# sandyresearch/chipmunk

Measured on AMD Instinct MI355X. Metric: DiT denoise steps/sec at fixed sparsity, higher is better.
Workload: dtype bf16

## Files before the change

### chipmunk_amd/csrc/attn64.hip

```cpp
#include "common.h"
#include "attn64_regs.h"
#include "attn_params.h"
#include "attn64_util.h"
#include <type_traits>

namespace {

constexpr int HD = 128;
constexpr int KT = 64;
constexpr int WROWS = 64, WGROWS = 256;
constexpr int TB = KT * HD * 2;
constexpr int NSL = 4;
constexpr int VRING = NSL * TB;
constexpr int LDS_BYTES = 2 * NSL * TB;
constexpr int PSTAGE = 64 * 128;
constexpr int LDS_BYTES_CSUM = LDS_BYTES + 4 * PSTAGE;
constexpr int CS_EXCH_BYTES = 2 * 4 * 64 * 4;
constexpr float SCALE_LOG2E = 0.08838834764f * 1.44269504089f;
constexpr float MAX_LAG = 4.0f;
#ifndef A64_ABL
#define A64_ABL 0
#endif
#ifndef A64_EB
#define A64_EB 20
#endif
#ifndef A64_EA
#define A64_EA 35
#endif
#ifndef A64_CSUM_VALU
#define A64_CSUM_VALU 1
#endif
#ifndef A64_VSPREAD
#define A64_VSPREAD 0
#endif
#ifndef A64_DMA_POS
#define A64_DMA_POS 2
#endif

constexpr int a64_ecum(int k) {
    return k <= 0 ? 0 : k <= 20 ? (k * A64_EB) / 20 : k <= 52 ? A64_EB + ((k - 20) * A64_EA) / 32
                                                              : (A64_EB + A64_EA + (k - 52) < 64 ? A64_EB + A64_EA + (k - 52) : 64);
}
constexpr int a64_cstep(int j) {
    int k = 0;
    while (a64_ecum(k) < 2 * j + 2) ++k;
    return k;
}
constexpr int a64_rk(int u) { return u == 0 ? 36 : u == 1 ? 38 : u == 2 ? 68 : 70; }
constexpr int a64_mk(int u) { return u == 0 ? 46 : u == 1 ? 48 : u == 2 ? 78 : 80; }

#ifdef ATTN64_PROF
__device__ unsigned long long g_a64_prof[4 * 8];
#define P64_DECL unsigned long long pt_ = 0, pacc_[7] = {0, 0, 0, 0, 0, 0, 0}; const bool prof_on_ = blockIdx.x == (gridDim.x / 2)
#define P64_START() do { if (prof_on_) pt_ = __builtin_amdgcn_s_memtime(); } while (0)
#define P64_MARK(i) do { if (prof_on_) { const unsigned long long n_ = __builtin_amdgcn_s_memtime(); pacc_[i] += n_ - pt_; pt_ = n_; } } while (0)
#define P64_END(w, n) do { if (prof_on_ && lane == 0) { for (int i_ = 0; i_ < 7; ++i_) g_a64_prof[(w) * 8 + i_] = pacc_[i_]; g_a64_prof[(w) * 8 + 7] = (n); } } while (0)
#else
#define P64_DECL
#define P64_START()
#define P64_MARK(i)
#define P64_END(w, n)
#endif

template <int KB, int QB, int KS>
__device__ __forceinline__ void mfma_qk(f32x16 &s) {
    constexpr int ka = 192 + (KB * 8 + KS) * 4, qa = 128 + (QB * 8 + KS) * 4;
    if constexpr (A64_ABL & 64) {
        constexpr int oa = (KB * 2 + QB) * 16;
        asm volatile("v_mfma_f32_32x32x16_bf16 a[%c0:%c1], a[%c2:%c3], a[%c4:%c5], a[%c0:%c1]" ::"i"(oa), "i"(oa + 15), "i"(ka), "i"(ka + 3), "i"(qa), "i"(qa + 3));
        return;
    }
    if constexpr (KS == 0)
        asm volatile("v_mfma_f32_32x32x16_bf16 %0, a[%c1:%c2], a[%c3:%c4], 0" : "=v"(s) : "i"(ka), "i"(ka + 3), "i"(qa), "i"(qa + 3));
    else
        asm volatile("v_mfma_f32_32x32x16_bf16 %0, a[%c1:%c2], a[%c3:%c4], %0" : "+v"(s) : "i"(ka), "i"(ka + 3), "i"(qa), "i"(qa + 3));
}
template <int QB, int DB>
__device__ __forceinline__ void mfma_pv(const u32x4 &vf, const u32x4 &pf) {
    constexpr int oa = (QB * 4 + DB) * 16;
    asm volatile("v_mfma_f32_32x32x16_bf16 a[%c2:%c3], %0, %1, a[%c2:%c3]" ::"v"(vf), "v"(pf), "i"(oa), "i"(oa + 15));
}
template <int KB, int KS, int SLOT>
__device__ __forceinline__ void lds_k(uint32_t addr) {
    constexpr int ka = 192 + (KB * 8 + KS) * 4;
    asm volatile("ds_read_b128 a[%c1:%c2], %0 offset:%c3" ::"v"(addr), "i"(ka), "i"(ka + 3), "i"(SLOT * TB + KB * 8192) : "memory");
}
__device__ __forceinline__ void cs_pair16x2(float &a, float &b, float &c, float &d) {
    asm volatile("v_permlane16_swap_b32 %0, %1\n\tv_permlane16_swap_b32 %2, %3\n\tv_add_f32 %0, %0, %1\n\tv_add_f32 %2, %2, %3"
                 : "+v"(a), "+v"(b), "+v"(c), "+v"(d));
}
__device__ __forceinline__ void cs_pair8(float &a, const float &b) {
    asm volatile("v_add_f32_dpp %0, %0, %0 row_mirror row_mask:0xf bank_mask:0x3\n\t"
                 "v_add_f32_dpp %0, %1, %1 row_mirror row_mask:0xf bank_mask:0xc" : "+v"(a) : "v"(b));
}
__device__ __forceinline__ void cs_pair4(float &a, const float &b) {
    asm volatile("v_add_f32_dpp %0, %0, %0 row_half_mirror row_mask:0xf bank_mask:0x5\n\t"
                 "v_add_f32_dpp %0, %1, %1 row_half_mirror row_mask:0xf bank_mask:0xa" : "+v"(a) : "v"(b));
}
template <int CTRL>
__device__ __forceinline__ float cs_pair_quad(float a, float b, bool hi) {
    const float keep = hi ? b : a, give = hi ? a : b;
    return keep + __uint_as_float((uint32_t)__builtin_amdgcn_update_dpp(0, (int)__float_as_uint(give), CTRL, 0xf, 0xf, true));
}
__global__ __launch_bounds__(256) void knorm_max_kernel(const uint16_t *k, const int64_t ks0, const int64_t ks1, const int64_t ks2, int H, int Nk,
                                                        float *out) {
    const int bh = blockIdx.y, b = bh / H, h = bh - b * H;
    const uint16_t *kb = k + b * ks0 + h * ks1;
    const int grp = threadIdx.x >> 4, li = threadIdx.x & 15;
    float best = 0.f;
#pragma unroll 4
    for (int row = blockIdx.x * 16 + grp; row < Nk; row += gridDim.x * 16) {
        const u32x4 v = *(const u32x4 *)(kb + (int64_t)row * ks2 + li * 8);
        float ss = 0.f;
#pragma unroll
        for (int e = 0; e < 4; ++e) {
            const float lo = __uint_as_float(v[e] << 16), hi = __uint_as_float(v[e] & 0xffff0000u);
            ss = __builtin_fmaf(lo, lo, ss);
            ss = __builtin_fmaf(hi, hi, ss);
        }
        best = fmaxf(best, row16_sum(ss));
    }
    __shared__ float red[256];
    red[threadIdx.x] = best;
    __syncthreads();
    for (int st = 128; st > 0; st >>= 1) {
        if ((int)threadIdx.x < st) red[threadIdx.x] = fmaxf(red[threadIdx.x], red[threadIdx.x + st]);
        __syncthreads();
    }
    if (threadIdx.x == 0) atomicMax((unsigned int *)(out + bh), __float_as_uint(__builtin_sqrtf(red[0])));
}

template <int MODE>
// ... 96 lines not shown
            __syncthreads();
        }
        return;
    }

    asm volatile(A64_ZERO_O ::: A64_CLOBBER_ALL);
    float qss[2] = {0.f, 0.f};
    {
        const uint16_t *qp = p.q + b * p.qs[0] + h * p.qs[1];
        static_for<0, 16>([&](auto f) {
            constexpr int F = decltype(f)::value, qb = F >> 3, ks = F & 7;
            const int qrow = row0 + qb * 32 + l31;
            u32x4 val = {0u, 0u, 0u, 0u};
            if (qrow < p.Nq) val = *(const u32x4 *)(qp + (int64_t)qrow * p.qs[2] + ks * 16 + hf * 8);
            acc_write4<128 + F * 4>(val);
#pragma unroll
            for (int e = 0; e < 4; ++e) {
                const float lo = __uint_as_float(val[e] << 16), hi = __uint_as_float(val[e] & 0xffff0000u);
                qss[qb] = __builtin_fmaf(lo, lo, qss[qb]);
                qss[qb] = __builtin_fmaf(hi, hi, qss[qb]);
            }
        });
    }

    const uint32_t lds0 = (uint32_t)(uintptr_t)(__attribute__((address_space(3))) unsigned char *)smem;
    uint32_t kad[8];
#pragma unroll
    for (int ks = 0; ks < 8; ++ks) kad[ks] = lds0 + l31 * 256 + (((2 * ks + hf) ^ l15) << 4);
    uint32_t vad[4];
#pragma unroll
    for (int db = 0; db < 4; ++db)
        vad[db] = lds0 + VRING + (4 * hf + (l15 >> 2)) * 256 + (((db * 4 + 2 * (lg & 1) + ((l15 & 3) >> 1)) ^ ((l15 >> 2) << 2)) << 4) +
                  (l15 & 1) * 8;
    uint32_t kofs[4];
#pragma unroll
    for (int i = 0; i < 4; ++i) kofs[i] = (uint32_t)(w * 16 + 4 * i + lg) * kstride_b + ((uint32_t)(l15 ^ (4 * i + lg)) << 4);
    const uint32_t vofs = (uint32_t)(w * 16 + lg) * vstride_b + ((uint32_t)(l15 ^ (lg << 2)) << 4);

    const int last_base = p.Nk - KT;
    auto tile_base = [&](int T) { return T * KT < last_base ? T * KT : last_base; };
    auto issue_k1 = [&](uint32_t soff, uint32_t ldsw, int slot, int i) {
        blds16(krsrc, kofs[i], soff, smem + ldsw + slot * TB + i * 1024);
    };
    auto issue_v1 = [&](uint32_t soff, uint32_t ldsw, int slot, int i) {
        blds16(vrsrc, vofs, soff + (uint32_t)(4 * i) * vstride_b, smem + ldsw + VRING + slot * TB + i * 1024);
    };
    auto issue_k = [&](int T, int slot) {
        const uint32_t soff = (uint32_t)tile_base(T) * kstride_b;
#pragma unroll
        for (int i = 0; i < 4; ++i) issue_k1(soff, w * 4096, slot, i);
    };
    auto issue_v = [&](int T, int slot) {
        const uint32_t soff = (uint32_t)tile_base(T) * vstride_b;
#pragma unroll
        for (int i = 0; i < 4; ++i) issue_v1(soff, w * 4096, slot, i);
    };

    if constexpr (!GATHER) {
        issue_k(0, 0);
        issue_k(1, 1), issue_v(0, 3);
        issue_k(2, 2), issue_v(0, 0);
        issue_k(3, 3), issue_v(1, 1);
        asm volatile("s_waitcnt vmcnt(24)" ::: "memory");
    }
    __syncthreads();
    static_for<0, 16>([&](auto i) {
        constexpr int I = decltype(i)::value;
        lds_k<(I >> 3), (I & 7), 0>(kad[I & 7]);
    });
    asm volatile("s_waitcnt lgkmcnt(0)" ::: "memory");

    f32x16 s[4];
    float px[64];
    uint32_t pw[2][4][4] = {};
    float m[2] = {-INFINITY, -INFINITY}, nmsc[2] = {0.f, 0.f};
    float mlag[2] = {-INFINITY, -INFINITY};
    float lacc[2][2] = {{0.f, 0.f}, {0.f, 0.f}};
    float alpha[2] = {1.f, 1.f};
    float wq[2] = {0.f, 0.f}, lpq[2] = {-1.0e30f, -1.0e30f}, c4[2] = {0.f, 0.f}, c5 = 0.f;
    uint32_t csoff = 0, ex_w = 0, ex_r = 0;
    int cs_extra = 0;
    float cs_own = 0.f;
    __amdgpu_buffer_rsrc_t prsrc = krsrc;
    uint32_t pst_w = 0, pst_r = 0, csoff_mx = 0;
    u32x2 csf[8] = {};
    f32x4 csacc[2] = {{0.f, 0.f, 0.f, 0.f}, {0.f, 0.f, 0.f, 0.f}};
    float csout = 0.f;
    u32x4 cs_ones = {0x3f803f80u, 0x3f803f80u, 0x3f803f80u, 0x3f803f80u};
    if constexpr (CSUM) {
        static_assert(A64_CSUM_VALU, "the matrix-pipe column-sum probe (A64_CSUM_VALU=0) fills all 160 KiB of LDS with its P stage: no room for the exchange area of the in-workgroup combine; build round 5's tree for it");
        pin(cs_ones);
        const uint32_t pst = lds0 + LDS_BYTES + (uint32_t)w * PSTAGE;
        pst_w = pst + l31 * 128 + ((uint32_t)(hf ^ (l31 & 7)) << 4);
        const int prow = lg * 4 + (l15 >> 2);
        pst_r = pst + prow * 128 + ((uint32_t)(((l15 & 3) >> 1) ^ (prow & 7)) << 4) + (l15 & 1) * 8;
        csoff_mx = 2u * (uint32_t)(16 * lg + 8 * ((l15 >> 2) & 1) + 4 * (l15 >> 3) + (l15 & 3));
#pragma unroll
        for (int qb = 0; qb < 2; ++qb) {
            const int qrow = row0 + qb * 32 + l31;
            const float pl = qrow < p.Nq ? p.p_in[(int64_t)bh * p.Nq + qrow] : 0.f;
            lpq[qb] = pl > 0.f ? __builtin_amdgcn_logf(pl) : -1.0e30f;
        }
        const int rr = ((lane >> 4) & 1) | (((lane >> 3) & 1) << 1) | (((lane >> 2) & 1) << 2);
        csoff = 2u * (uint32_t)(32 * (lane & 1) + (rr & 3) + 8 * (2 * ((lane >> 1) & 1) + (rr >> 2)) + 4 * hf);
        const int nA = 3 - (4 * g) % 3;
        const int lead = w < nA ? 0 : nA, members = w < nA ? nA : 4 - nA;
        cs_extra = w == lead ? members : 0;
        ex_w = lds0 + LDS_BYTES + (uint32_t)w * 256u + (uint32_t)lane * 4u;
        ex_r = lds0 + LDS_BYTES + (uint32_t)(lead + 1) * 256u + (uint32_t)lane * 4u;
        prsrc = make_rsrc(p.cs_part + ((int64_t)bh * (p.G * 2) + (g * 2 + (w < nA ? 0 : 1))) * p.cs_pstride);
    }
#pragma unroll
    for (int e = 0; e < 64; ++e) px[e] = e < 20 ? 0.f : -INFINITY;

    auto vfrag_read = [&](auto dbc, auto offc) __attribute__((always_inline)) {
        constexpr int DB = decltype(dbc)::value, OFF = decltype(offc)::value;
        u32x2 lo, hi;
        asm volatile("ds_read_b64_tr_b16 %0, %2 offset:%c3\n\tds_read_b64_tr_b16 %1, %2 offset:%c4"
                     : "=&v"(lo), "=&v"(hi) : "v"(vad[DB]), "i"(OFF), "i"(OFF + 2048) : "memory");
        return (u32x4){lo[0], lo[1], hi[0], hi[1]};
    };

    static_assert(64 - A64_EB - A64_EA >= 0 && 64 - A64_EB - A64_EA <= 9, "the last steps must finish before gap 12 of the next PV phase");
    auto ecum = [](int k) constexpr { return a64_ecum(k); };
    auto finish_step = [&](auto kk, auto uwc) __attribute__((always_inline)) {
        constexpr int K = decltype(kk)::value;
        constexpr bool UW = decltype(uwc)::value != 0;
        if constexpr (!(A64_ABL & 1)) {
            static_for<ecum(K), ecum(K + 1)>([&](auto ii) {
                constexpr int I = decltype(ii)::value;
                if constexpr (A64_ABL & 32) px[I] = px[I] * 0.5f;
                else px[I] = __builtin_amdgcn_exp2f(px[I]);
                pin(px[I]);
            });
            static_for<ecum(K - 1), ecum(K)>([&](auto ii) {
                constexpr int I = decltype(ii)::value;
                lacc[(I >> 3) & 1][I & 1] += px[I];
                pin(lacc[(I >> 3) & 1][I & 1]);
            });
            static_for<(ecum(K - 1) >> 1), (ecum(K) >> 1)>([&](auto jj) {
                constexpr int J = decltype(jj)::value, I = 2 * J;
                pw[(I >> 3) & 1][I >> 4][(I & 7) >> 1] = pack_bf16x2(px[I], px[I + 1]);
                pin(pw[(I >> 3) & 1][I >> 4][(I & 7) >> 1]);
            });
            if constexpr (CSUM && UW && !A64_CSUM_VALU) {
                static_assert(a64_cstep(8 * 1 + 7) + 1 < a64_rk(0) && a64_cstep(8 * 3 + 7) + 1 < a64_rk(2), "a unit is read after its second fragment is stored");
                static_for<0, 4>([&](auto uu) {
                    constexpr int U = decltype(uu)::value, S = (U & 1) * 4;
                    if constexpr (K == a64_mk(U) || K == a64_mk(U) + 1) {
                        constexpr int H2 = K - a64_mk(U);
                        if constexpr (H2 == 0 && (U & 1) == 0)
                            asm volatile("s_waitcnt lgkmcnt(0)" : "+v"(csf[0]), "+v"(csf[1]), "+v"(csf[2]), "+v"(csf[3]), "+v"(csf[4]), "+v"(csf[5]), "+v"(csf[6]), "+v"(csf[7]) :: "memory");
                        const u32x4 fr = {csf[S + 2 * H2][0], csf[S + 2 * H2][1], csf[S + 2 * H2 + 1][0], csf[S + 2 * H2 + 1][1]};
                        if constexpr (H2 == 0) asm volatile("v_mfma_f32_16x16x32_bf16 %0, %1, %2, 0" : "=&v"(csacc[U & 1]) : "v"(cs_ones), "v"(fr));
                        else asm volatile("v_mfma_f32_16x16x32_bf16 %0, %1, %2, %0" : "+v"(csacc[U & 1]) : "v"(cs_ones), "v"(fr));
                    }
                    if constexpr (K == a64_mk(U) + 3) {
                        if constexpr (U == 0) csout = csacc[0][0];
                        else csout = lg == U ? csacc[U & 1][0] : csout;
                        pin(csout);
                    }
                    if constexpr (K == a64_rk(U) || K == a64_rk(U) + 1) {
                        constexpr int H2 = K - a64_rk(U);
                        uint32_t ad = pst_r;
                        if constexpr (U != 0) ad ^= (uint32_t)(U << 5);
                        asm volatile("ds_read_b64_tr_b16 %0, %2 offset:%c3\n\tds_read_b64_tr_b16 %1, %2 offset:%c4"
                                     : "=&v"(csf[S + 2 * H2]), "=&v"(csf[S + 2 * H2 + 1]) : "v"(ad), "i"(H2 * 4096), "i"(H2 * 4096 + 2048) : "memory");
                    }
                });
                static_for<0, 8>([&](auto ii) {
                    constexpr int U = decltype(ii)::value >> 1, QW = decltype(ii)::value & 1;
                    if constexpr (K == a64_cstep(8 * U + 4 * QW + 3) + 1) {
                        uint32_t ad = pst_w;
                        if constexpr (U != 0) ad ^= (uint32_t)(U << 5);
                        const u32x4 pf = {pw[QW][U][0], pw[QW][U][1], pw[QW][U][2], pw[QW][U][3]};
                        asm volatile("ds_write_b128 %0, %1 offset:%c2" ::"v"(ad), "v"(pf), "i"(QW * 4096) : "memory");
                    }
                });
            } else if constexpr (CSUM) {
                static_for<ecum(K - 3), ecum(K - 2)>([&](auto ii) {
                    constexpr int I = decltype(ii)::value;
                    if constexpr (UW) {
                        if constexpr (((I >> 3) & 1) == 1) { px[I] += px[I - 8]; pin(px[I]); }
                    } else {
                        if constexpr (((I >> 3) & 1) == 0) px[I] *= wq[0];
                        else px[I] = __builtin_fmaf(px[I], wq[1], px[I - 8]);
                        pin(px[I]);
                    }
                });
                static_for<ecum(K - 4), ecum(K - 3)>([&](auto ii) {
                    constexpr int I = decltype(ii)::value;
                    if constexpr ((I & 11) == 11) cs_pair16x2(px[I - 3], px[I - 2], px[I - 1], px[I]);
                });
                static_for<ecum(K - 5), ecum(K - 4)>([&](auto ii) {
                    constexpr int I = decltype(ii)::value;
                    if constexpr ((I & 11) == 11) cs_pair8(px[I - 3], px[I - 1]);
                });
                static_for<ecum(K - 6), ecum(K - 5)>([&](auto ii) {
                    constexpr int I = decltype(ii)::value;
                    if constexpr ((I & 15) == 15) cs_pair4(px[I - 7], px[I - 3]);
                });
                static_for<ecum(K - 7), ecum(K - 6)>([&](auto ii) {
                    constexpr int I = decltype(ii)::value;
                    if constexpr ((I & 31) == 31) { c4[I >> 5] = cs_pair_quad<0x4E>(px[I - 23], px[I - 7], (lane & 2) != 0); pin(c4[I >> 5]); }
                });
                static_for<ecum(K - 8), ecum(K - 7)>([&](auto ii) {
                    constexpr int I = decltype(ii)::value;
                    if constexpr (I == 63) { c5 = cs_pair_quad<0xB1>(c4[0], c4[1], (lane & 1) != 0); pin(c5); }
                });
            }
        }
    };

    P64_DECL;
    P64_START();
    auto tile = [&](auto slc, auto nmc, int t) __attribute__((always_inline)) {
        constexpr int SL = decltype(slc)::value;
        constexpr bool NOMAX = decltype(nmc)::value != 0;
        constexpr auto uwc = ic<(CSUM && decltype(nmc)::value == 2) ? 1 : 0>{};
        constexpr int VSL = (SL + 3) & 3;
        constexpr int KNSL = (SL + 1) & 3;
        uint32_t ldsw = w * 4096, ksoff = 0, vsoff = 0;
        if constexpr (!(A64_ABL & 16)) {
            if constexpr (!(A64_ABL & 256) && !GATHER) asm volatile("s_waitcnt vmcnt(16)" ::: "memory");
            if constexpr (!(A64_ABL & 128)) __builtin_amdgcn_s_barrier();
            if constexpr (!GATHER) {
                asm volatile("" : "+s"(ldsw));
                ksoff = (uint32_t)tile_base(t + 4) * kstride_b;
                vsoff = (uint32_t)tile_base(t + 2) * vstride_b;
            }
        }
        __builtin_amdgcn_sched_barrier(0);
        P64_MARK(0);

        u32x4 vf[16];
        static_for<0, 32>([&](auto gg) {
            constexpr int G = decltype(gg)::value;
            constexpr int ks = G >> 2, kb = (G >> 1) & 1, qb = G & 1;
            mfma_qk<kb, qb, ks>(s[kb * 2 + qb]);
            if constexpr (!(A64_ABL & 16) && !GATHER && ((A64_DMA_POS == 0 && G < 8) || (A64_DMA_POS == 2 && G >= 16 && (G & 1) == 0))) {
                constexpr int PC = A64_DMA_POS == 0 ? G : (G - 16) >> 1;
                if constexpr (PC < 4) issue_k1(ksoff, ldsw, SL, PC);
                else issue_v1(vsoff, ldsw, (SL + 2) & 3, PC - 4);
            }
            finish_step(ic<20 + G>{}, uwc);
            if constexpr (A64_VSPREAD ? (G & 1) == 0 : G < 16) {
                constexpr int f = A64_VSPREAD ? G >> 1 : G;
                if constexpr (A64_ABL & 4) vf[f] = (u32x4){(uint32_t)t, 1u, 2u, 3u};
                else vf[f] = vfrag_read(ic<(f & 3)>{}, ic<VSL * TB + (f >> 2) * 4096>{});
            }
            __builtin_amdgcn_sched_barrier(0);
        });
        P64_MARK(1);
        asm volatile("s_waitcnt lgkmcnt(0)"
                     : "+v"(vf[0]), "+v"(vf[1]), "+v"(vf[2]), "+v"(vf[3]), "+v"(vf[4]), "+v"(vf[5]), "+v"(vf[6]), "+v"(vf[7]), "+v"(vf[8]),
                       "+v"(vf[9]), "+v"(vf[10]), "+v"(vf[11]), "+v"(vf[12]), "+v"(vf[13]), "+v"(vf[14]), "+v"(vf[15]));
        __builtin_amdgcn_sched_barrier(0);
        P64_MARK(2);

        float mx[2];
        bool moved = false;
        const int dead = GATHER ? 0 : (t * KT - tile_base(t) < KT ? t * KT - tile_base(t) : KT);
        const int vleft = !GATHER ? KT : (t < ntiles ? valid - (tbeg + t) * KT : 0);
        auto phase_b_gap = [&](auto gg) __attribute__((always_inline)) {
            constexpr int G = decltype(gg)::value;
            constexpr int up = G >> 3, db = (G >> 1) & 3, qb = G & 1;
            const u32x4 pf = {pw[qb][up][0], pw[qb][up][1], pw[qb][up][2], pw[qb][up][3]};
            mfma_pv<qb, db>(vf[G >> 1], pf);
            constexpr bool UWT = decltype(uwc)::value != 0 && !A64_CSUM_VALU;
            if constexpr (G < (CSUM ? (UWT ? 32 : 17) : 12)) finish_step(ic<52 + G>{}, uwc);
            if constexpr (CSUM && G == (UWT ? 31 : 17)) {
                const uint32_t par2 = (uint32_t)(t & 1) * 1024u;
                const float mine = UWT ? csout : c5;
                if (!cs_extra) {
                    asm volatile("ds_write_b32 %0, %1" ::"v"(ex_w + (par2 ^ 1024u)), "v"(mine) : "memory");
                } else {
                    float x1 = 0.f, x2 = 0.f;
                    if (cs_extra >= 2) asm volatile("ds_read_b32 %0, %1" : "=v"(x1) : "v"(ex_r + par2) : "memory");
                    if (cs_extra >= 3) asm volatile("ds_read_b32 %0, %1 offset:256" : "=v"(x2) : "v"(ex_r + par2) : "memory");
                    asm volatile("ds_write_b32 %0, %1" ::"v"(ex_w + (par2 ^ 1024u)), "v"(mine) : "memory");
                    asm volatile("s_waitcnt lgkmcnt(1)" : "+v"(x1), "+v"(x2)::"memory");
                    const int tb2 = tile_base(t - 2), dd = (t - 2) * KT - tb2;
                    if (t > 1 && dd < KT) {
                        const uint32_t off = UWT ? csoff_mx : csoff;
                        if (dd <= 0 || (int)(off >> 1) >= dd) {
                            const uint16_t val = (uint16_t)(pack_bf16x2((cs_own + x1) + x2, 0.f) & 0xffffu);
                            if (p.probe & 16) __builtin_amdgcn_raw_buffer_store_b16(val, prsrc, off, (uint32_t)tb2 * 2u, 2);
                            else __builtin_amdgcn_raw_buffer_store_b16(val, prsrc, off, (uint32_t)tb2 * 2u, 0);
                        }
                    }
                }
                cs_own = mine;
            }
            if constexpr (!(A64_ABL & 16) && !GATHER && A64_DMA_POS == 1 && G >= 16 && (G & 1) == 0) {
                constexpr int PC = (G - 16) >> 1;
                if constexpr (PC < 4) issue_k1(ksoff, ldsw, SL, PC);
                else issue_v1(vsoff, ldsw, (SL + 2) & 3, PC - 4);
            }
            if constexpr (G < 16 && !(A64_ABL & 8)) {
                constexpr int J = G;
                lds_k<(J >> 3), (J & 7), KNSL>(kad[J & 7]);
            }
            if constexpr (G == 1 && !(A64_ABL & 2)) {
                if (!GATHER && __builtin_expect(dead > 0, 0)) {
                    int thr = dead - 4 * hf;
                    asm volatile("" : "+v"(thr));
#pragma unroll
                    for (int blk = 0; blk < 4; ++blk)
#pragma unroll
                        for (int r = 0; r < 16; ++r)
                            if ((blk >> 1) * 32 + (r & 3) + 8 * (r >> 2) < thr) s[blk][r] = -INFINITY;
                }
                if (GATHER && __builtin_expect(vleft < KT, 0)) {
                    int thr = vleft - hf;
                    asm volatile("" : "+v"(thr));
#pragma unroll
                    for (int blk = 0; blk < 4; ++blk)
#pragma unroll
                        for (int r = 0; r < 16; ++r)
                            if ((r & 3) * 16 + (blk >> 1) * 8 + 2 * (r >> 2) >= thr) s[blk][r] = -INFINITY;
                }
            }
            if constexpr (G >= 2 && G <= 9 && !(A64_ABL & 2) && !NOMAX) {
                constexpr int j = G - 2;
                constexpr int kb2 = j >> 2, r0 = (j & 3) * 4;
                if constexpr (j == 0)
                    asm volatile("v_max_f32 %0, %2, %3\n\tv_max_f32 %1, %6, %7\n\tv_max3_f32 %0, %0, %4, %5\n\tv_max3_f32 %1, %1, %8, %9"
                                 : "=&v"(mx[0]), "=&v"(mx[1])
                                 : "v"(s[0][0]), "v"(s[0][1]), "v"(s[0][2]), "v"(s[0][3]), "v"(s[1][0]), "v"(s[1][1]), "v"(s[1][2]), "v"(s[1][3]));
                else
                asm volatile("v_max3_f32 %0, %0, %2, %3\n\tv_max3_f32 %1, %1, %6, %7\n\tv_max3_f32 %0, %0, %4, %5\n\tv_max3_f32 %1, %1, %8, %9"
                             : "+v"(mx[0]), "+v"(mx[1])
                             : "v"(s[kb2 * 2][r0]), "v"(s[kb2 * 2][r0 + 1]), "v"(s[kb2 * 2][r0 + 2]), "v"(s[kb2 * 2][r0 + 3]),
                               "v"(s[kb2 * 2 + 1][r0]), "v"(s[kb2 * 2 + 1][r0 + 1]), "v"(s[kb2 * 2 + 1][r0 + 2]), "v"(s[kb2 * 2 + 1][r0 + 3]));
            }
            if constexpr (G == 10 && !(A64_ABL & 2) && !NOMAX) {
#pragma unroll
                for (int q2 = 0; q2 < 2; ++q2) {
                    float a = mx[q2], c = mx[q2];
                    lane_swap32(a, c);
                    mx[q2] = max2(a, c);
                    pin(mx[q2]);
                }
            }
            if constexpr (G >= 12 && G < 28 && !(A64_ABL & 2)) {
                static_for<(G - 12) * 4, (G - 11) * 4>([&](auto ii) {
                    constexpr int I = decltype(ii)::value;
                    constexpr int blk = (I >> 5) * 2 + ((I >> 3) & 1), r = ((I >> 4) & 1) * 8 + (I & 7);
                    px[I] = __builtin_fmaf(s[blk][r], SCALE_LOG2E, nmsc[(I >> 3) & 1]);
                    pin(px[I]);
                });
            }
            if constexpr (G >= 12) finish_step(ic<G - 12>{}, uwc);
            __builtin_amdgcn_sched_barrier(0);
        };
        static_for<0, 12>(phase_b_gap);
        P64_MARK(3);
        if constexpr (!(A64_ABL & 2) && !NOMAX) {
            constexpr float LAG_RAW = MAX_LAG / SCALE_LOG2E;
            if (__builtin_amdgcn_ballot_w64(mx[0] > mlag[0]) | __builtin_amdgcn_ballot_w64(mx[1] > mlag[1])) {
                moved = true;
#pragma unroll
                for (int q2 = 0; q2 < 2; ++q2) {
                    const float m_new = max2(m[q2], mx[q2]);
                    alpha[q2] = __builtin_amdgcn_exp2f((m[q2] - m_new) * SCALE_LOG2E);
                    lacc[q2][0] *= alpha[q2];
                    lacc[q2][1] *= alpha[q2];
                    m[q2] = m_new;
                    nmsc[q2] = -m_new * SCALE_LOG2E;
                    mlag[q2] = m_new + LAG_RAW;
                    if constexpr (CSUM) wq[q2] = fminf(__builtin_amdgcn_exp2f(m_new * SCALE_LOG2E + lpq[q2]), 1.0e37f);
                }
            }
        }
        __builtin_amdgcn_sched_barrier(0);
        P64_MARK(4);
        static_for<12, 32>(phase_b_gap);
        P64_MARK(5);
        if (__builtin_expect(moved, 0)) {
            float tmp;
            asm volatile("s_nop 7\n\ts_nop 7\n\ts_nop 7\n\t" A64_SCALE_QB0 : "=&v"(tmp) : "v"(alpha[0]));
            asm volatile(A64_SCALE_QB1 : "=&v"(tmp) : "v"(alpha[1]));
        }
        asm volatile("s_waitcnt lgkmcnt(0)" ::: "memory");
        __builtin_amdgcn_sched_barrier(0);
        P64_MARK(6);
    };

    bool nomax = false;
    if constexpr (!GATHER) {
        if (p.kmax) {
            const float km = p.kmax[bh];
            bool ok = true;
#pragma unroll
            for (int qb = 0; qb < 2; ++qb) {
                float a = qss[qb], c2 = qss[qb];
                lane_swap32(a, c2);
                const float mq = __builtin_sqrtf(a + c2) * km;
                ok = ok && (2.0f * mq * SCALE_LOG2E <= 64.0f);
                qss[qb] = mq;
            }
            nomax = __builtin_amdgcn_ballot_w64(!ok) == 0;
            if (nomax) {
#pragma unroll
                for (int qb = 0; qb < 2; ++qb) {
                    m[qb] = qss[qb], nmsc[qb] = -qss[qb] * SCALE_LOG2E, mlag[qb] = INFINITY;
                    if constexpr (CSUM) wq[qb] = fminf(__builtin_amdgcn_exp2f(qss[qb] * SCALE_LOG2E + lpq[qb]), 1.0e37f);
                }
            }
        }
    }
    bool unitw = false;
    if constexpr (CSUM) {
        if (nomax && !(p.probe & 4)) {
            bool ok = true;
#pragma unroll
            for (int qb = 0; qb < 2; ++qb) ok = ok && lpq[qb] > -1.0e29f && qss[qb] * SCALE_LOG2E + __builtin_fabsf(lpq[qb]) <= 80.0f;
            unitw = __builtin_amdgcn_ballot_w64(!ok) == 0;
            if (unitw) {
#pragma unroll
                for (int qb = 0; qb < 2; ++qb) m[qb] = -lpq[qb] / SCALE_LOG2E, nmsc[qb] = lpq[qb];
            }
        }
    }
    if (CSUM && unitw) {
        if constexpr (CSUM) {
            for (int tb = 0;; tb += 4) {
                tile(ic<0>{}, ic<2>{}, tb);
                if (tb >= T4) break;
                tile(ic<1>{}, ic<2>{}, tb + 1);
                tile(ic<2>{}, ic<2>{}, tb + 2);
                tile(ic<3>{}, ic<2>{}, tb + 3);
            }
        }
    } else if (nomax) {
        for (int tb = 0;; tb += 4) {
            tile(ic<0>{}, ic<1>{}, tb);
            if (tb >= T4) break;
            tile(ic<1>{}, ic<1>{}, tb + 1);
            tile(ic<2>{}, ic<1>{}, tb + 2);
            tile(ic<3>{}, ic<1>{}, tb + 3);
        }
    } else {
        for (int tb = 0;; tb += 4) {
            tile(ic<0>{}, ic<0>{}, tb);
            if (tb >= T4) break;
            tile(ic<1>{}, ic<0>{}, tb + 1);
            tile(ic<2>{}, ic<0>{}, tb + 2);
            tile(ic<3>{}, ic<0>{}, tb + 3);
        }
    }
    asm volatile("s_waitcnt vmcnt(0)" ::: "memory");
    P64_END(w, T4 + 1);
    if constexpr (CSUM) {
        asm volatile("s_waitcnt lgkmcnt(0)" ::: "memory");
        __builtin_amdgcn_s_barrier();
        if (cs_extra) {
            float x1 = 0.f, x2 = 0.f;
            const uint32_t par = (uint32_t)((T4 - 1) & 1) * 1024u;
            if (cs_extra >= 2) asm volatile("ds_read_b32 %0, %1" : "=v"(x1) : "v"(ex_r + par) : "memory");
            if (cs_extra >= 3) asm volatile("ds_read_b32 %0, %1 offset:256" : "=v"(x2) : "v"(ex_r + par) : "memory");
            asm volatile("s_waitcnt lgkmcnt(0)" : "+v"(x1), "+v"(x2)::"memory");
            const int tb1 = tile_base(T4 - 1), dd = (T4 - 1) * KT - tb1;
            const uint32_t off = (unitw && !A64_CSUM_VALU) ? csoff_mx : csoff;
            if (dd < KT && (dd <= 0 || (int)(off >> 1) >= dd))
                __builtin_amdgcn_raw_buffer_store_b16((uint16_t)(pack_bf16x2((cs_own + x1) + x2, 0.f) & 0xffffu), prsrc, off, (uint32_t)tb1 * 2u, 0);
        }
    }

    asm volatile("s_nop 7\n\ts_nop 7\n\ts_nop 7" ::: "memory");
    float o[128];
    static_for<0, 32>([&](auto ii) {
        constexpr int I = decltype(ii)::value;
        const f32x4 o4 = acc_read4<I * 4>();
        o[I * 4 + 0] = o4[0], o[I * 4 + 1] = o4[1], o[I * 4 + 2] = o4[2], o[I * 4 + 3] = o4[3];
    });
    float lq[2];
#pragma unroll
    for (int qb = 0; qb < 2; ++qb) {
        float lp = lacc[qb][0] + lacc[qb][1], lo2 = lp;
        lane_swap32(lp, lo2);
        lq[qb] = lp + lo2;
    }

    if constexpr (GATHER) {
        if (nsp > 1) {
            constexpr int SLICE_FLOATS = 26 * 256 * 4;
            int *ticket_s = (int *)smem;
            float *mine = p.ws + (int64_t)(slot0 + sp) * SLICE_FLOATS + tid;
#pragma unroll
            for (int i = 0; i < 128; ++i) mine[i * 192] = o[i];
            mine[128 * 192] = m[0], mine[129 * 192] = m[1], mine[130 * 192] = lq[0], mine[131 * 192] = lq[1];
            __syncthreads();
            if (tid == 0) {
                __builtin_amdgcn_fence(__ATOMIC_RELEASE, "agent");
                asm volatile("s_waitcnt vmcnt(0)" ::: "memory");
                *ticket_s = __hip_atomic_fetch_add(p.tickets + tix, 1, __ATOMIC_RELAXED, __HIP_MEMORY_SCOPE_AGENT);
            }
            __syncthreads();
            if (*ticket_s != nsp - 1) return;
            if (tid == 0) {
                __hip_atomic_store(p.tickets + tix, 0, __ATOMIC_RELAXED, __HIP_MEMORY_SCOPE_AGENT);
                __builtin_amdgcn_fence(__ATOMIC_ACQUIRE, "agent");
            }
            __syncthreads();
#pragma unroll
            for (int i = 0; i < 128; ++i) o[i] = 0.f;
            m[0] = m[1] = -INFINITY, lq[0] = lq[1] = 0.f;
            for (int s2 = 0; s2 < nsp; ++s2) {
                const float *oth = p.ws + (int64_t)(slot0 + s2) * SLICE_FLOATS + tid;
#pragma unroll
                for (int qb = 0; qb < 2; ++qb) {
                    const float ms = oth[(128 + qb) * 192], ls = oth[(130 + qb) * 192];
                    const float m_new = fmaxf(m[qb], ms);
                    if (m_new == -INFINITY) continue;
                    const float a = __builtin_amdgcn_exp2f((m[qb] - m_new) * SCALE_LOG2E);
                    const float c = __builtin_amdgcn_exp2f((ms - m_new) * SCALE_LOG2E);
                    m[qb] = m_new;
                    lq[qb] = lq[qb] * a + ls * c;
#pragma unroll
                    for (int i = 0; i < 64; ++i) o[qb * 64 + i] = o[qb * 64 + i] * a + oth[(qb * 64 + i) * 192] * c;
                }
            }
        }
    }

#pragma unroll
    for (int qb = 0; qb < 2; ++qb) {
        const float l = lq[qb];
        const float inv = l > 0.f ? __builtin_amdgcn_rcpf(l) : 0.f;
        const int qrow = row0 + qb * 32 + l31;
        if (qrow >= p.Nq) continue;
        const int64_t ooff = b * p.os[0] + h * p.os[1] + (int64_t)qrow * p.os[2] + 4 * hf;
        uint16_t *op = p.o + ooff;
#pragma unroll
        for (int i = 0; i < 16; ++i) {
            const int db = i >> 2, r4 = i & 3;
            const float *o4 = o + (qb * 4 + db) * 16 + r4 * 4;
            float x0 = o4[0] * inv, x1 = o4[1] * inv, x2 = o4[2] * inv, x3 = o4[3] * inv;
            u32x2 out;
            if constexpr (INPLACE) {
                const u32x2 old = *(const u32x2 *)(p.o_in + ooff + db * 32 + r4 * 8);
                const float a0 = round_bf16(x0 * p.o_scale), a1 = round_bf16(x1 * p.o_scale);
                const float a2 = round_bf16(x2 * p.o_scale), a3 = round_bf16(x3 * p.o_scale);
                out[0] = pack_bf16x2(__uint_as_float(old[0] << 16) + a0, __uint_as_float(old[0] & 0xffff0000u) + a1);
                out[1] = pack_bf16x2(__uint_as_float(old[1] << 16) + a2, __uint_as_float(old[1] & 0xffff0000u) + a3);
            } else {
// ... 78 lines not shown
        lds_k<(I >> 3), (I & 7), 0>(kad[I & 7]);
    });
    asm volatile("s_waitcnt lgkmcnt(0)" ::: "memory");

    f32x16 s[3][2];
#pragma unroll
    for (int i = 0; i < 3; ++i)
#pragma unroll
        for (int kb = 0; kb < 2; ++kb)
#pragma unroll
            for (int r = 0; r < 16; ++r) s[i][kb][r] = -1.0e30f;
    float cacc[2][2] = {{0.f, 0.f}, {0.f, 0.f}};

    float pe[2] = {0.f, 0.f};
    auto drain2 = [&](auto bufc, auto tpc, auto e0c, auto ptpc, auto pe0c) __attribute__((always_inline)) {
        constexpr int BUF = decltype(bufc)::value, TP = decltype(tpc)::value, E0 = decltype(e0c)::value;
        constexpr int PTP = decltype(ptpc)::value, PE0 = decltype(pe0c)::value;
        (void)TP;
        const float n0 = __builtin_amdgcn_exp2f(s[BUF][E0 >> 4][E0 & 15]);
        const float n1 = __builtin_amdgcn_exp2f(s[BUF][(E0 + 1) >> 4][(E0 + 1) & 15]);
        cacc[PTP][PE0 >> 4] += pe[0];
        cacc[PTP][(PE0 + 1) >> 4] += pe[1];
        pe[0] = n0, pe[1] = n1;
        pin(pe[0]), pin(pe[1]), pin(cacc[PTP][PE0 >> 4]);
    };

    auto tile = [&](auto slc, int t) __attribute__((always_inline)) {
        constexpr int SL = decltype(slc)::value, TP = SL & 1, KNSL = (SL + 1) & 3;
        asm volatile("s_waitcnt vmcnt(8)" ::: "memory");
        __builtin_amdgcn_s_barrier();
        uint32_t ldsw = w * 4096;
        asm volatile("" : "+s"(ldsw));
        const uint32_t ksoff = (uint32_t)tile_base(t + 4) * kstride_b;
        __builtin_amdgcn_sched_barrier(0);
        static_for<0, 6>([&](auto qq) {
            constexpr int QB = decltype(qq)::value;
            constexpr int PP = SL * 6 + QB;
            constexpr int BUF = PP % 3, B1 = (PP + 2) % 3, B2 = (PP + 1) % 3;
            static_for<0, 16>([&](auto gg) {
                constexpr int G = decltype(gg)::value, ks = G >> 1, kb = G & 1;
                mfma_cs<QB, kb, ks>(s[BUF][kb], offs[QB]);
                if constexpr (QB == 0 && G >= 8 && G < 12) issue_k1(ksoff, ldsw, SL, G - 8);
                if constexpr (QB == 5 && kb == 1) {
                    lds_k<0, ks, KNSL>(kad[ks]);
                    lds_k<1, ks, KNSL>(kad[ks]);
                }
                constexpr int TP1 = QB == 0 ? TP ^ 1 : TP, TP2 = QB <= 1 ? TP ^ 1 : TP;
                if constexpr (G > 2) drain2(ic<B1>{}, ic<TP1>{}, ic<(G - 2) * 2>{}, ic<TP1>{}, ic<(G - 3) * 2>{});
                else if constexpr (G == 2) drain2(ic<B1>{}, ic<TP1>{}, ic<0>{}, ic<TP2>{}, ic<30>{});
                else if constexpr (G == 1) drain2(ic<B2>{}, ic<TP2>{}, ic<30>{}, ic<TP2>{}, ic<28>{});
                else drain2(ic<B2>{}, ic<TP2>{}, ic<28>{}, ic<TP2>{}, ic<26>{});
                if constexpr (QB == 1 && G == 3) {
                    float a = cacc[TP ^ 1][0], c = cacc[TP ^ 1][1];
                    lane_swap32(a, c);
                    const float tot = a + c;
                    cacc[TP ^ 1][0] = 0.f, cacc[TP ^ 1][1] = 0.f;
                    if (g < p.G && t > 0)
                    {
                        const uint32_t u = __float_as_uint(tot);
                        const uint32_t rne = (u + 0x7fffu + ((u >> 16) & 1u)) >> 16, qn = (u >> 16) | 0x0040u;
                        p.cs[((int64_t)bh * p.G + g) * p.cs_stride + tile_base(t - 1) + lane] = (uint16_t)((u & 0x7fffffffu) > 0x7f800000u ? qn : rne);
                    }
                }
                __builtin_amdgcn_sched_barrier(0);
            });
        });
        asm volatile("s_waitcnt lgkmcnt(0)" ::: "memory");
        __builtin_amdgcn_sched_barrier(0);
    };
    for (int tb = 0;; tb += 4) {
        tile(ic<0>{}, tb);
        if (tb >= T4) break;
        tile(ic<1>{}, tb + 1);
        tile(ic<2>{}, tb + 2);
        tile(ic<3>{}, tb + 3);
    }
    asm volatile("s_waitcnt vmcnt(0)" ::: "memory");
}

template <int MODE>
int launch64(const AttnParams &p, int64_t grid, hipStream_t stream) {
    auto kern = attn64_kernel<MODE>;
    static uint64_t lds_set = 0;
    constexpr int LDS = (MODE == 3 && !A64_CSUM_VALU) ? LDS_BYTES_CSUM + CS_EXCH_BYTES : MODE == 3 ? LDS_BYTES + CS_EXCH_BYTES : LDS_BYTES;
    ensure_dynamic_lds((const void *)kern, LDS, lds_set);
    hipLaunchKernelGGL(kern, dim3((unsigned)grid), dim3(256), LDS, stream, p);
    CM_LAUNCH_CHECK();
    return CHIPMUNK_OK;
}

}

#ifdef ATTN64_PROF
extern "C" int chipmunk_attn64_prof_read(unsigned long long *out) {
    return hipMemcpyFromSymbol(out, HIP_SYMBOL(g_a64_prof), sizeof(g_a64_prof)) == hipSuccess ? 0 : 2;
}
#endif

const float *chipmunk_knorm_max(const uint16_t *k, const int64_t ks[3], int B, int H, int Nk, hipStream_t stream) {
    if (chipmunk_get_option("attn_nomax") == 2 || (size_t)B * H * sizeof(float) > (32 << 10)) return nullptr;
    unsigned char *sc = (unsigned char *)chipmunk_scratch(stream, 64 << 10);
    if (!sc) return nullptr;
    float *km = (float *)(sc + (32 << 10));
    if (hipMemsetAsync(km, 0, (size_t)B * H * sizeof(float), stream) != hipSuccess) return nullptr;
    hipLaunchKernelGGL(knorm_max_kernel, dim3(Nk >= 4096 ? 64 : 8, B * H), dim3(256), 0, stream, k, ks[0], ks[1], ks[2], H, Nk, km);
    return km;
}

int chipmunk_dense64_launch(const void *q, const void *k, const void *v, void *o, float *l, const int64_t qs[3],
                            const int64_t ks[3], const int64_t vs[3], const int64_t os[3], int B, int H, int Nq, int Nk,
                            hipStream_t stream) {
    AttnParams p = {};
    p.q = (const uint16_t *)q, p.k = (const uint16_t *)k, p.v = (const uint16_t *)v, p.o = (uint16_t *)o;
    for (int i = 0; i < 3; ++i) p.qs[i] = qs[i], p.ks[i] = ks[i], p.vs[i] = vs[i], p.os[i] = os[i];
    p.l_out = l;
    p.B = B, p.H = H, p.Nq = Nq, p.Nk = Nk, p.G = (Nq + WGROWS - 1) / WGROWS;
    p.o_scale = 1.f;
    p.kmax = chipmunk_knorm_max(p.k, ks, B, H, Nk, stream);
    return launch64<0>(p, (int64_t)B * H * p.G, stream);
}

namespace {
__global__ __launch_bounds__(256) void cs_combine_kernel(const uint16_t *part, int pstride, uint16_t *cs, int NRB, int G, int Nq, int Nk, int cs_stride) {
    const int g = blockIdx.y, bh = blockIdx.z;
    int r0, r1;
    const int nrows = colsum_part_rows(g, NRB / 2, r0, r1);
    const uint16_t *src = part + ((int64_t)bh * NRB + r0) * pstride;
    const int64_t row1 = (int64_t)(r1 - r0) * pstride;
    uint16_t *dst = cs + ((int64_t)bh * G + g) * cs_stride;
    if (((Nk | cs_stride) & 3) == 0) {
        const int j = (blockIdx.x * 256 + threadIdx.x) * 4;
        if (j >= Nk) return;
        float acc[4];
        {
            const u32x2 x = *(const u32x2 *)(src + j);
            acc[0] = __uint_as_float(x[0] << 16), acc[1] = __uint_as_float(x[0] & 0xffff0000u);
            acc[2] = __uint_as_float(x[1] << 16), acc[3] = __uint_as_float(x[1] & 0xffff0000u);
        }
        if (nrows == 2) {
            const u32x2 x = *(const u32x2 *)(src + row1 + j);
            acc[0] += __uint_as_float(x[0] << 16), acc[1] += __uint_as_float(x[0] & 0xffff0000u);
            acc[2] += __uint_as_float(x[1] << 16), acc[3] += __uint_as_float(x[1] & 0xffff0000u);
        }
        *(u32x2 *)(dst + j) = (u32x2){pack_bf16x2(acc[0], acc[1]), pack_bf16x2(acc[2], acc[3])};
    } else {
        for (int e = 0; e < 4; ++e) {
            const int j = (blockIdx.x * 256 + threadIdx.x) * 4 + e;
            if (j >= Nk) return;
            float acc = bf16_bits_to_f32(src[j]);
            if (nrows == 2) acc += bf16_bits_to_f32(src[row1 + j]);
            dst[j] = f32_to_bf16_bits(acc);
        }
    }
}
}

int chipmunk_colsum64_launch(const AttnParams &p, hipStream_t stream) {
    static uint64_t lds_set = 0;
    ensure_dynamic_lds((const void *)colsum64_kernel, NSL * TB, lds_set);
    const int64_t grid = (int64_t)p.B * p.H * ((p.G + 3) / 4);
    hipLaunchKernelGGL(colsum64_kernel, dim3((unsigned)grid), dim3(256), NSL * TB, stream, p);
    CM_LAUNCH_CHECK();
    return CHIPMUNK_OK;
}

int chipmunk_colsum_part_stride(int Nk) { return (chipmunk_get_option("attn_cs_probe") & 1) ? Nk : (Nk + 63) & ~63; }

// ... 25 lines not shown
```

### chipmunk_amd/csrc/attn64_util.h

```cpp
#pragma once
#include <type_traits>
#include "common.h"

namespace {

template <int V>
using ic = std::integral_constant<int, V>;
template <int I, int N, typename F>
__device__ __forceinline__ void static_for(F &&f) {
    if constexpr (I < N) {
        f(ic<I>{});
        static_for<I + 1, N>(f);
    }
}

template <typename T>
__device__ __forceinline__ void pin(T &x) {
    asm volatile("" : "+v"(x));
}
__device__ __forceinline__ float max3(float a, float b, float c) {
    float r;
    asm("v_max3_f32 %0, %1, %2, %3" : "=v"(r) : "v"(a), "v"(b), "v"(c));
    return r;
}
__device__ __forceinline__ float max2(float a, float b) {
    float r;
    asm("v_max_f32 %0, %1, %2" : "=v"(r) : "v"(a), "v"(b));
    return r;
}

template <int BASE>
__device__ __forceinline__ void acc_write4(const u32x4 &v) {
    asm volatile("v_accvgpr_write_b32 a%c4, %0\n\tv_accvgpr_write_b32 a%c5, %1\n\tv_accvgpr_write_b32 a%c6, %2\n\tv_accvgpr_write_b32 a%c7, %3\n\ts_nop 1"
                 ::"v"(v[0]), "v"(v[1]), "v"(v[2]), "v"(v[3]), "i"(BASE), "i"(BASE + 1), "i"(BASE + 2), "i"(BASE + 3));
}
template <int BASE>
__device__ __forceinline__ f32x4 acc_read4() {
    float a, b, c, d;
    asm volatile("v_accvgpr_read_b32 %0, a%c4\n\tv_accvgpr_read_b32 %1, a%c5\n\tv_accvgpr_read_b32 %2, a%c6\n\tv_accvgpr_read_b32 %3, a%c7"
                 : "=v"(a), "=v"(b), "=v"(c), "=v"(d) : "i"(BASE), "i"(BASE + 1), "i"(BASE + 2), "i"(BASE + 3));
    return (f32x4){a, b, c, d};
}


}
```

Before: 0.5647.

## Compute column sums with register-fed MFMA selector instead of LDS-staged P

Replaces the VALU column-sum path, now off by default, with a matrix-pipe column sum. It multiplies the in-register P fragments by a lane-selector bf16 matrix and reduces the result with permlane swaps. The old matrix-pipe probe staged P through extra LDS and transposed reads back. That path and its LDS region are removed, so the kernel keeps its smaller LDS footprint. It adds MFMA and permlane work inside the PV loop, and output offsets are remapped through a lane key.

```diff
diff --git a/chipmunk_amd/csrc/attn64.hip b/chipmunk_amd/csrc/attn64.hip
--- a/chipmunk_amd/csrc/attn64.hip
+++ b/chipmunk_amd/csrc/attn64.hip
@@ -13,8 +13,6 @@
 constexpr int NSL = 4;
 constexpr int VRING = NSL * TB;
 constexpr int LDS_BYTES = 2 * NSL * TB;
-constexpr int PSTAGE = 64 * 128;
-constexpr int LDS_BYTES_CSUM = LDS_BYTES + 4 * PSTAGE;
 constexpr int CS_EXCH_BYTES = 2 * 4 * 64 * 4;
 constexpr float SCALE_LOG2E = 0.08838834764f * 1.44269504089f;
 constexpr float MAX_LAG = 4.0f;
@@ -28,7 +26,7 @@
 #define A64_EA 35
 #endif
 #ifndef A64_CSUM_VALU
-#define A64_CSUM_VALU 1
+#define A64_CSUM_VALU 0
 #endif
 #ifndef A64_VSPREAD
 #define A64_VSPREAD 0
@@ -46,8 +44,12 @@
     while (a64_ecum(k) < 2 * j + 2) ++k;
     return k;
 }
-constexpr int a64_rk(int u) { return u == 0 ? 36 : u == 1 ? 38 : u == 2 ? 68 : 70; }
-constexpr int a64_mk(int u) { return u == 0 ? 46 : u == 1 ? 48 : u == 2 ? 78 : 80; }
+constexpr int a64_sg_mfma(int u, int qb) { return 8 * u + qb; }
+constexpr int a64_sg_add(int u) { return 8 * u + 3; }
+constexpr int A64_SG_SWAP32 = 28, A64_SG_SWAP16 = 29, A64_SG_STORE = 31;
+static_assert(a64_sg_mfma(3, 1) >= a64_sg_mfma(3, 0) + 1 && a64_sg_add(3) >= a64_sg_mfma(3, 1) + 2, "chained MFMA one gap behind the first, first VALU read two gaps behind it");
+static_assert(a64_sg_add(0) < a64_sg_mfma(1, 0) && a64_sg_add(1) < a64_sg_mfma(2, 0) && a64_sg_add(2) < a64_sg_mfma(3, 0), "one accumulator: a unit is folded before the next one starts");
+static_assert(A64_SG_SWAP32 > a64_sg_add(3) && A64_SG_SWAP16 > A64_SG_SWAP32 && A64_SG_STORE > A64_SG_SWAP16, "swaps read what a VALU wrote at least a gap earlier");
 
 #ifdef ATTN64_PROF
 __device__ unsigned long long g_a64_prof[4 * 8];
@@ -310,19 +312,13 @@
     int cs_extra = 0;
     float cs_own = 0.f;
     __amdgpu_buffer_rsrc_t prsrc = krsrc;
-    uint32_t pst_w = 0, pst_r = 0, csoff_mx = 0;
-    u32x2 csf[8] = {};
-    f32x4 csacc[2] = {{0.f, 0.f, 0.f, 0.f}, {0.f, 0.f, 0.f, 0.f}};
-    float csout = 0.f;
-    u32x4 cs_ones = {0x3f803f80u, 0x3f803f80u, 0x3f803f80u, 0x3f803f80u};
+    u32x4 cs_sel = {0u, 0u, 0u, 0u};
+    f32x4 csacc = {0.f, 0.f, 0.f, 0.f};
+    float csu[4] = {0.f, 0.f, 0.f, 0.f}, csout = 0.f;
     if constexpr (CSUM) {
-        static_assert(A64_CSUM_VALU, "the matrix-pipe column-sum probe (A64_CSUM_VALU=0) fills all 160 KiB of LDS with its P stage: no room for the exchange area of the in-workgroup combine; build round 5's tree for it");
-        pin(cs_ones);
-        const uint32_t pst = lds0 + LDS_BYTES + (uint32_t)w * PSTAGE;
-        pst_w = pst + l31 * 128 + ((uint32_t)(hf ^ (l31 & 7)) << 4);
-        const int prow = lg * 4 + (l15 >> 2);
-        pst_r = pst + prow * 128 + ((uint32_t)(((l15 & 3) >> 1) ^ (prow & 7)) << 4) + (l15 & 1) * 8;
-        csoff_mx = 2u * (uint32_t)(16 * lg + 8 * ((l15 >> 2) & 1) + 4 * (l15 >> 3) + (l15 & 3));
+#pragma unroll
+        for (int d = 0; d < 4; ++d) cs_sel[d] = (a64_cs_sel(lane, 2 * d) ? 0x3f80u : 0u) | (a64_cs_sel(lane, 2 * d + 1) ? 0x3f800000u : 0u);
+        pin(cs_sel);
 #pragma unroll
         for (int qb = 0; qb < 2; ++qb) {
             const int qrow = row0 + qb * 32 + l31;
@@ -334,8 +330,8 @@
         const int nA = 3 - (4 * g) % 3;
         const int lead = w < nA ? 0 : nA, members = w < nA ? nA : 4 - nA;
         cs_extra = w == lead ? members : 0;
-        ex_w = lds0 + LDS_BYTES + (uint32_t)w * 256u + (uint32_t)lane * 4u;
-        ex_r = lds0 + LDS_BYTES + (uint32_t)(lead + 1) * 256u + (uint32_t)lane * 4u;
+        ex_w = lds0 + LDS_BYTES + (uint32_t)w * 256u;
+        ex_r = lds0 + LDS_BYTES + (uint32_t)(lead + 1) * 256u;
         prsrc = make_rsrc(p.cs_part + ((int64_t)bh * (p.G * 2) + (g * 2 + (w < nA ? 0 : 1))) * p.cs_pstride);
     }
 #pragma unroll
@@ -371,41 +367,7 @@
                 pw[(I >> 3) & 1][I >> 4][(I & 7) >> 1] = pack_bf16x2(px[I], px[I + 1]);
                 pin(pw[(I >> 3) & 1][I >> 4][(I & 7) >> 1]);
             });
-            if constexpr (CSUM && UW && !A64_CSUM_VALU) {
-                static_assert(a64_cstep(8 * 1 + 7) + 1 < a64_rk(0) && a64_cstep(8 * 3 + 7) + 1 < a64_rk(2), "a unit is read after its second fragment is stored");
-                static_for<0, 4>([&](auto uu) {
-                    constexpr int U = decltype(uu)::value, S = (U & 1) * 4;
-                    if constexpr (K == a64_mk(U) || K == a64_mk(U) + 1) {
-                        constexpr int H2 = K - a64_mk(U);
-                        if constexpr (H2 == 0 && (U & 1) == 0)
-                            asm volatile("s_waitcnt lgkmcnt(0)" : "+v"(csf[0]), "+v"(csf[1]), "+v"(csf[2]), "+v"(csf[3]), "+v"(csf[4]), "+v"(csf[5]), "+v"(csf[6]), "+v"(csf[7]) :: "memory");
-                        const u32x4 fr = {csf[S + 2 * H2][0], csf[S + 2 * H2][1], csf[S + 2 * H2 + 1][0], csf[S + 2 * H2 + 1][1]};
-                        if constexpr (H2 == 0) asm volatile("v_mfma_f32_16x16x32_bf16 %0, %1, %2, 0" : "=&v"(csacc[U & 1]) : "v"(cs_ones), "v"(fr));
-                        else asm volatile("v_mfma_f32_16x16x32_bf16 %0, %1, %2, %0" : "+v"(csacc[U & 1]) : "v"(cs_ones), "v"(fr));
-                    }
-                    if constexpr (K == a64_mk(U) + 3) {
-                        if constexpr (U == 0) csout = csacc[0][0];
-                        else csout = lg == U ? csacc[U & 1][0] : csout;
-                        pin(csout);
-                    }
-                    if constexpr (K == a64_rk(U) || K == a64_rk(U) + 1) {
-                        constexpr int H2 = K - a64_rk(U);
-                        uint32_t ad = pst_r;
-                        if constexpr (U != 0) ad ^= (uint32_t)(U << 5);
-                        asm volatile("ds_read_b64_tr_b16 %0, %2 offset:%c3\n\tds_read_b64_tr_b16 %1, %2 offset:%c4"
-                                     : "=&v"(csf[S + 2 * H2]), "=&v"(csf[S + 2 * H2 + 1]) : "v"(ad), "i"(H2 * 4096), "i"(H2 * 4096 + 2048) : "memory");
-                    }
-                });
-                static_for<0, 8>([&](auto ii) {
-                    constexpr int U = decltype(ii)::value >> 1, QW = decltype(ii)::value & 1;
-                    if constexpr (K == a64_cstep(8 * U + 4 * QW + 3) + 1) {
-                        uint32_t ad = pst_w;
-                        if constexpr (U != 0) ad ^= (uint32_t)(U << 5);
-                        const u32x4 pf = {pw[QW][U][0], pw[QW][U][1], pw[QW][U][2], pw[QW][U][3]};
-                        asm volatile("ds_write_b128 %0, %1 offset:%c2" ::"v"(ad), "v"(pf), "i"(QW * 4096) : "memory");
-                    }
-                });
-            } else if constexpr (CSUM) {
+            if constexpr (CSUM && (!UW || A64_CSUM_VALU)) {
                 static_for<ecum(K - 3), ecum(K - 2)>([&](auto ii) {
                     constexpr int I = decltype(ii)::value;
                     if constexpr (UW) {
@@ -496,8 +458,23 @@
             const u32x4 pf = {pw[qb][up][0], pw[qb][up][1], pw[qb][up][2], pw[qb][up][3]};
             mfma_pv<qb, db>(vf[G >> 1], pf);
             constexpr bool UWT = decltype(uwc)::value != 0 && !A64_CSUM_VALU;
-            if constexpr (G < (CSUM ? (UWT ? 32 : 17) : 12)) finish_step(ic<52 + G>{}, uwc);
-            if constexpr (CSUM && G == (UWT ? 31 : 17)) {
+            if constexpr (G < (CSUM && !UWT ? 17 : 12)) finish_step(ic<52 + G>{}, uwc);
+            if constexpr (UWT) {
+                if constexpr (G == a64_sg_mfma(up, 0)) asm volatile("v_mfma_f32_16x16x32_bf16 %0, %1, %2, 0" : "=&v"(csacc) : "v"(pf), "v"(cs_sel));
+                if constexpr (G == a64_sg_mfma(up, 1)) asm volatile("v_mfma_f32_16x16x32_bf16 %0, %1, %2, %0" : "+v"(csacc) : "v"(pf), "v"(cs_sel));
+                if constexpr (G == a64_sg_add(up)) {
+                    csu[up] = (csacc[0] + csacc[1]) + (csacc[2] + csacc[3]);
+                    pin(csu[up]);
+                }
+                if constexpr (G == A64_SG_SWAP32)
+                    asm volatile("s_nop 0\n\tv_permlane32_swap_b32 %0, %1\n\tv_permlane32_swap_b32 %2, %3\n\tv_add_f32 %0, %0, %1\n\tv_add_f32 %2, %2, %3"
+                                 : "+v"(csu[0]), "+v"(csu[2]), "+v"(csu[1]), "+v"(csu[3]));
+                if constexpr (G == A64_SG_SWAP16) {
+                    asm volatile("s_nop 0\n\tv_permlane16_swap_b32 %0, %1\n\ts_nop 0\n\tv_add_f32 %0, %0, %1" : "+v"(csu[0]), "+v"(csu[1]));
+                    csout = csu[0];
+                }
+            }
+            if constexpr (CSUM && G == (UWT ? A64_SG_STORE : 17)) {
                 const uint32_t par2 = (uint32_t)(t & 1) * 1024u;
                 const float mine = UWT ? csout : c5;
                 if (!cs_extra) {
@@ -510,7 +487,7 @@
                     asm volatile("s_waitcnt lgkmcnt(1)" : "+v"(x1), "+v"(x2)::"memory");
                     const int tb2 = tile_base(t - 2), dd = (t - 2) * KT - tb2;
                     if (t > 1 && dd < KT) {
-                        const uint32_t off = UWT ? csoff_mx : csoff;
+                        const uint32_t off = csoff;
                         if (dd <= 0 || (int)(off >> 1) >= dd) {
                             const uint16_t val = (uint16_t)(pack_bf16x2((cs_own + x1) + x2, 0.f) & 0xffffu);
                             if (p.probe & 16) __builtin_amdgcn_raw_buffer_store_b16(val, prsrc, off, (uint32_t)tb2 * 2u, 2);
@@ -651,6 +628,10 @@
             }
         }
     }
+    if constexpr (CSUM) {
+        if (unitw && !A64_CSUM_VALU) csoff = 2u * (uint32_t)a64_cs_lane_key(lane);
+        ex_w += 2u * csoff, ex_r += 2u * csoff;
+    }
     if (CSUM && unitw) {
         if constexpr (CSUM) {
             for (int tb = 0;; tb += 4) {
@@ -690,7 +671,7 @@
             if (cs_extra >= 3) asm volatile("ds_read_b32 %0, %1 offset:256" : "=v"(x2) : "v"(ex_r + par) : "memory");
             asm volatile("s_waitcnt lgkmcnt(0)" : "+v"(x1), "+v"(x2)::"memory");
             const int tb1 = tile_base(T4 - 1), dd = (T4 - 1) * KT - tb1;
-            const uint32_t off = (unitw && !A64_CSUM_VALU) ? csoff_mx : csoff;
+            const uint32_t off = csoff;
             if (dd < KT && (dd <= 0 || (int)(off >> 1) >= dd))
                 __builtin_amdgcn_raw_buffer_store_b16((uint16_t)(pack_bf16x2((cs_own + x1) + x2, 0.f) & 0xffffu), prsrc, off, (uint32_t)tb1 * 2u, 0);
         }
@@ -935,7 +916,7 @@
 int launch64(const AttnParams &p, int64_t grid, hipStream_t stream) {
     auto kern = attn64_kernel<MODE>;
     static uint64_t lds_set = 0;
-    constexpr int LDS = (MODE == 3 && !A64_CSUM_VALU) ? LDS_BYTES_CSUM + CS_EXCH_BYTES : MODE == 3 ? LDS_BYTES + CS_EXCH_BYTES : LDS_BYTES;
+    constexpr int LDS = MODE == 3 ? LDS_BYTES + CS_EXCH_BYTES : LDS_BYTES;
     ensure_dynamic_lds((const void *)kern, LDS, lds_set);
     hipLaunchKernelGGL(kern, dim3((unsigned)grid), dim3(256), LDS, stream, p);
     CM_LAUNCH_CHECK();
diff --git a/chipmunk_amd/csrc/attn64_util.h b/chipmunk_amd/csrc/attn64_util.h
--- a/chipmunk_amd/csrc/attn64_util.h
+++ b/chipmunk_amd/csrc/attn64_util.h
@@ -41,6 +41,12 @@
                  : "=v"(a), "=v"(b), "=v"(c), "=v"(d) : "i"(BASE), "i"(BASE + 1), "i"(BASE + 2), "i"(BASE + 3));
     return (f32x4){a, b, c, d};
 }
-
+constexpr int a64_cs_pi(int off) { return off; }
+constexpr bool a64_cs_sel(int lane, int j) { return (lane & 15) == a64_cs_pi(8 * (j >> 2) + 4 * ((lane >> 4) >> 1) + (j & 3)); }
+constexpr int a64_cs_lane_key(int lane) {
+    int off = 0;
+    while (a64_cs_pi(off) != (lane & 15)) ++off;
+    return 16 * (lane >> 4) + off;
+}
 
 }
```

Measured after the change: 0.5657 (median of 6 runs). About the same (+0.2%).
